# iris-ua/iris_lama

Measured on NVIDIA H100. Metric: scans/sec at 256 particles x 1080 beams, higher is better.
Workload: dtype f64

## Files before the change

iris_lama_b200/csrc/brushfire_warp.cuh:

```cuda
#pragma once

#include "ddm_core.h"
#include "device_store.cuh"

namespace lama_b200 {

constexpr unsigned kFullMask = 0xffffffffu;

struct SmemHeap {
    uint64_t* slot;
    uint32_t size, cap;

    __device__ __forceinline__ bool push(uint64_t value)
    {
        if (size >= cap) return false;
        int hole = (int)size++;
        while (hole > 0) {
            int parent = (hole - 1) >> 1;
            uint64_t pv = slot[parent + 1];
            if (!heap_comp(pv, value)) break;
            slot[hole + 1] = pv;
            hole = parent;
        }
        slot[hole + 1] = value;
        return true;
    }
    __device__ __forceinline__ uint64_t top() const { return slot[1]; }
    __device__ __forceinline__ uint64_t pop()
    {
        const uint64_t t = slot[1];
        const uint32_t last = --size;
        if (last == 0) return t;
        const uint64_t value = slot[last + 1];
        const int len = (int)last;
        int hole = 0, second = 0;
        const int lim = (len - 1) >> 1;
        while (second < lim) {
            second = 2 * (second + 1);
            const ulonglong2 ch = *reinterpret_cast<const ulonglong2*>(slot + second);
            uint64_t pick = ch.y;
            if (heap_comp(ch.y, ch.x)) {
                pick = ch.x;
                second--;
            }
            slot[hole + 1] = pick;
            hole = second;
        }
        if ((len & 1) == 0 && second == ((len - 2) >> 1)) {
            second = 2 * (second + 1);
            slot[hole + 1] = slot[second];
            hole = second - 1;
        }
        while (hole > 0) {
            int parent = (hole - 1) >> 1;
            uint64_t pv = slot[parent + 1];
            if (!heap_comp(pv, value)) break;
            slot[hole + 1] = pv;
            hole = parent;
        }
        slot[hole + 1] = value;
        return t;
    }
};

struct WarpBrushfire {
    const StoreView& s;
    int32_t* dir;
    int32_t* gdir;
    uint32_t* scratch;
    const uint32_t side;
    const int log2dim;
    const int lane;
    SmemHeap lower_q, raise_q;
    const uint32_t max_sqdist;
    uint32_t err;
    bool dead;
#ifdef LAMA_PHASE_TIMING
    long long cyc[6] = {0, 0, 0, 0, 0, 0};
#define BF_CLK(v) const long long v = clock64()
#define BF_ACC(k, a, b) cyc[k] += (b) - (a)
#else
#define BF_CLK(v) do { } while (0)
#define BF_ACC(k, a, b) do { } while (0)
#endif

    __device__ WarpBrushfire(const StoreView& sv, int32_t* d, int32_t* g, uint32_t* sc, int l, SmemHeap lo, SmemHeap ra, uint32_t msq)
        : s(sv), dir(d), gdir(g), scratch(sc), side((uint32_t)sv.window.dim * kPatchLen), log2dim(ilog2(sv.window.dim)), lane(l), lower_q(lo),
          raise_q(ra), max_sqdist(msq), err(0), dead(false) {}

    __host__ __device__ static int ilog2(int v)
    {
        int l = 0;
        while ((1 << (l + 1)) <= v) ++l;
        return l;
    }
    __device__ __forceinline__ static uint32_t key_of(uint32_t x, uint32_t y) { return (y << 16) | (x & 0xFFFFu); }
    __device__ __forceinline__ int dindex(uint32_t x, uint32_t y) const
    {
        return (x < side && y < side) ? (int)(((y >> kPatchLog2) << log2dim) | (x >> kPatchLog2)) : -1;
    }
    __device__ __forceinline__ uint32_t* cellptr(int entry, uint32_t x, uint32_t y) const
    {
        return s.pool + ((((uint32_t)entry & (uint32_t)kDirSlotMask) << (2 * kPatchLog2)) | cell_index(x, y));
    }

    __device__ __forceinline__ bool entry_ready(int e) const { return e >= 0 && (e & kDirOwn); }

    __device__ __forceinline__ bool ensure(int di)
    {
        int slot = warp_make_exclusive(s, dir, gdir, di, lane);
        if (slot < 0) {
            err |= kErrPoolEmpty;
            dead = true;
            return false;
        }
        return true;
    }
    __device__ __forceinline__ uint32_t* uptr(uint32_t x, uint32_t y)
    {
        const int di = dindex(x, y);
        if (di < 0 || dead) {
            if (di < 0) err |= kErrWindow;
            scratch[lane] = 0;
            return &scratch[lane];
        }
        int e = dir[di];
        if (!entry_ready(e)) {
            if (!ensure(di)) {
                scratch[lane] = 0;
                return &scratch[lane];
            }
            e = dir[di];
        }
        return cellptr(e, x, y);
    }
    __device__ __forceinline__ uint32_t* lptr(uint32_t x, uint32_t y, bool active)
    {
        const int di = active ? dindex(x, y) : -1;
        if (active && di < 0) err |= kErrWindow;
        int e = di >= 0 ? dir[di] : -1;
        unsigned m = __ballot_sync(kFullMask, di >= 0 && !entry_ready(e));
        while (m && !dead) {
            const int l = __ffs(m) - 1;
            ensure(__shfl_sync(kFullMask, di, l));
            e = di >= 0 ? dir[di] : -1;
            m = __ballot_sync(kFullMask, di >= 0 && !entry_ready(e));
        }
        if (!entry_ready(e) || dead) {
            scratch[lane] = 0;
            return &scratch[lane];
        }
        return cellptr(e, x, y);
    }
    __device__ __forceinline__ static bool same_patch(uint32_t x, uint32_t y, int dx, int dy)
    {
        return (uint32_t)((int)(x & (kPatchLen - 1)) + dx) < (uint32_t)kPatchLen && (uint32_t)((int)(y & (kPatchLen - 1)) + dy) < (uint32_t)kPatchLen;
    }
    __device__ __forceinline__ uint32_t* rel_uptr(uint32_t* base, uint32_t x, uint32_t y, int dx, int dy)
    {
        if (same_patch(x, y, dx, dy) && !is_scratch(base)) return base + dx + dy * kPatchLen;
        return uptr(x + dx, y + dy);
    }
    __device__ __forceinline__ uint32_t* rel_lptr(uint32_t* base, bool interior, uint32_t x, uint32_t y, int dx, int dy, bool active)
    {
        if (interior && !is_scratch(base)) return active ? base + dx + dy * kPatchLen : &scratch[lane];
        return lptr(x + dx, y + dy, active);
    }
    __device__ __forceinline__ bool is_scratch(const uint32_t* p) const { return p >= scratch && p < scratch + 32; }
    __device__ __forceinline__ static bool interior_cell(uint32_t x, uint32_t y)
    {
        return ((x & (kPatchLen - 1)) - 1u) < (uint32_t)(kPatchLen - 2) && ((y & (kPatchLen - 1)) - 1u) < (uint32_t)(kPatchLen - 2);
    }

    __device__ __forceinline__ uint32_t touch(uint32_t* p)
    {
        uint32_t w = *p;
        if (!(w & kDmKnown)) {
            w |= kDmKnown;
            *p = w;
        }
        return w;
    }

    __device__ __forceinline__ void push_lower(uint32_t prio, uint32_t key)
    {
        if (!lower_q.push(heap_entry(prio, key))) err |= kErrHeapOverflow;
    }
    __device__ __forceinline__ void push_raise(uint32_t prio, uint32_t key)
    {
        if (!raise_q.push(heap_entry(prio, key))) err |= kErrHeapOverflow;
    }

    __device__ __forceinline__ void add_obstacle(uint32_t x, uint32_t y)
    {
        uint32_t* c = uptr(x, y);
        const uint32_t w = touch(c);
        if ((w & kDmValid) && dm_sqdist(w) == 0) return;
        *c = dm_pack(0, 0, 0, true, true);
        push_lower(0, key_of(x, y));
    }
    __device__ __forceinline__ void remove_obstacle(uint32_t x, uint32_t y)
    {
        uint32_t* c = uptr(x, y);
        const uint32_t w = touch(c);
        if (!((w & kDmValid) && dm_sqdist(w) == 0)) return;
        *c = dm_pack(0, 0, 0, false, true);
        push_raise(0, key_of(x, y));
    }

    __device__ __forceinline__ void raise(uint32_t x, uint32_t y, uint32_t* cur)
    {
        const int i = lane & 3;
        const bool act = lane < 4;
        const int dxi = (i == 0) - (i == 2), dyi = (i == 1) - (i == 3);
        const uint32_t nx = x + dxi, ny = y + dyi;
        uint32_t* p = rel_lptr(cur, interior_cell(x, y), x, y, dxi, dyi, act);
        uint32_t n = 0;
        if (act) n = touch(p);
        const bool go = act && !((n & kDmQueued) || !(n & kDmValid));
        uint32_t* po = lptr(nx + dm_ox(n), ny + dm_oy(n), go);
        if (go) touch(po);
        __syncwarp();
        const uint32_t key = key_of(nx, ny);
        for (int j = 0; j < 4; ++j) {
            uint32_t o = 0;
            if (lane == j && go) o = *po;
            const bool g   = __shfl_sync(kFullMask, (int)go, j) != 0;
            if (!g) continue;
            const bool clr = __shfl_sync(kFullMask, (int)!(o & kDmValid), j) != 0;
            const uint32_t k  = __shfl_sync(kFullMask, key, j);
            const uint32_t pr = __shfl_sync(kFullMask, dm_sqdist(n), j);
            if (clr) {
                push_raise(pr, k);
                if (lane == j) *p = dm_pack(0, 0, 0, false, true);
            } else {
                push_lower(pr, k);
                if (lane == j) *p = n | kDmQueued;
            }
            __syncwarp();
        }
        if (lane == 0) *cur &= ~kDmQueued;
        __syncwarp();
    }

    __device__ __forceinline__ void lower(uint32_t x, uint32_t y, uint32_t* cur, uint32_t c)
    {
        const int cox = dm_ox(c), coy = dm_oy(c);
        const int i = lane & 3;
        const int dxi = (i == 0) - (i == 2), dyi = (i == 1) - (i == 3);
        const bool go = lane < 4 && !(dxi * cox > 0 || dyi * coy > 0);
        const uint32_t nx = x + dxi, ny = y + dyi;
        BF_CLK(c0);
        uint32_t* p = rel_lptr(cur, interior_cell(x, y), x, y, dxi, dyi, go);
        uint32_t n = 0;
        if (go) n = touch(p);
#ifdef LAMA_PHASE_TIMING
        n = __shfl_sync(kFullMask, n, lane);
#endif
        BF_CLK(c1);
        BF_ACC(2, c0, c1);
        const int rx = cox - dxi, ry = coy - dyi;
        const uint32_t new_sq = (uint32_t)(rx * rx + ry * ry);
        const uint32_t cmp_sq = (n & kDmValid) ? dm_sqdist(n) : max_sqdist;
        bool over = go && new_sq < cmp_sq;
        const bool chk = go && !over && new_sq == dm_sqdist(n);
        if (__any_sync(kFullMask, chk)) {
            uint32_t* po = lptr(nx + dm_ox(n), ny + dm_oy(n), chk);
            if (chk) {
                const uint32_t o = touch(po);
                if (!(n & kDmValid) || !((o & kDmValid) && dm_sqdist(o) == 0)) over = true;
            }
        }
        __syncwarp();
        unsigned m = __ballot_sync(kFullMask, over) & 0xFu;
        BF_CLK(c2);
        BF_ACC(3, c1, c2);
        const uint32_t key = key_of(nx, ny);
        while (m) {
            const int l = __ffs(m) - 1;
            m &= m - 1;
            BF_CLK(c4);
            push_lower(__shfl_sync(kFullMask, new_sq, l), __shfl_sync(kFullMask, key, l));
            BF_CLK(c5);
            BF_ACC(5, c4, c5);
            if (lane == l) *p = dm_pack(new_sq, rx, ry, true, true);
        }
        if (lane == 0) *cur = c & ~kDmQueued;
        __syncwarp();
        BF_CLK(c3);
        BF_ACC(4, c2, c3);
    }

    __device__ __forceinline__ uint32_t update()
    {
        uint32_t processed = 0;
        while (raise_q.size) {
            const uint32_t key = heap_key(raise_q.pop());
            const uint32_t x = key & 0xFFFFu, y = key >> 16;
            uint32_t* cur = uptr(x, y);
            touch(cur);
            ++processed;
            raise(x, y, cur);
        }
        while (lower_q.size) {
            BF_CLK(a0);
            const uint32_t key = heap_key(lower_q.pop());
            BF_CLK(a1);
            BF_ACC(0, a0, a1);
            const uint32_t x = key & 0xFFFFu, y = key >> 16;
            uint32_t* cur = uptr(x, y);
            const uint32_t c = touch(cur);
            ++processed;
            if (c & kDmValid) {
                const uint32_t o = touch(rel_uptr(cur, x, y, dm_ox(c), dm_oy(c)));
                BF_CLK(a2);
                BF_ACC(1, a1, a2);
                if (dm_sqdist(o) == 0 && (c & kDmQueued)) lower(x, y, cur, c);
            }
        }
        return processed;
    }
};

}
```

iris_lama_b200/csrc/kernels.cu:

```cuda
#include "kernels.cuh"

#include <cstdio>

#include "brushfire_warp.cuh"

namespace lama_b200 {

namespace {

constexpr int kMatchThreads = 576;
constexpr int kRayThreads   = 512;

__device__ __forceinline__ double warp_sum(double v)
{
#pragma unroll
    for (int o = 16; o > 0; o >>= 1) v += __shfl_xor_sync(0xffffffffu, v, o);
    return v;
}

struct MatchShared {
    uint64_t bar;
    Affine tf;
    SE2 state;
    SolverControl ctl;
// ... 1048 lines not shown
    const RayPullView& pv = rp.pull;
    const RayPullLayout L(rp.scan.n_beams);
    PullCtaShared& sh   = *reinterpret_cast<PullCtaShared*>(smem_raw);
    PullEntry* list     = reinterpret_cast<PullEntry*>(smem_raw + L.list);
    uint32_t* hits      = reinterpret_cast<uint32_t*>(smem_raw + L.hits);
    PullWarpShared& w   = reinterpret_cast<PullWarpShared*>(smem_raw + L.warps)[warp];
    const RayPullHeader* hdr = &sh.hdr;
    const int dim = s.window.dim, S = pv.splits;
    int log2dim = 0;
    while ((1 << (log2dim + 1)) <= dim) ++log2dim;
    if (tid == 0) mbar_init(&sh.bar, 1);
    uint32_t err = 0, parity = 0;
    for (;;) {
        __syncthreads();
        if (tid == 0) sh.unit = atomicAdd(pv.ctrl + 1, 1);
        __syncthreads();
        const int unit = sh.unit;
        if (unit >= count * S) break;
        const int pl = unit / S, split = unit - pl * S;
        if (!__ldcg(&pv.hdr[pl].ok)) continue;
        if (tid == 0) {
            sh.hdr  = pv.hdr[pl];
            sh.next = 0;
            const uint32_t b0 = (uint32_t)sh.hdr.prefix[8] * (uint32_t)sizeof(PullEntry), b1 = ((uint32_t)sh.hdr.n_hits * 4u + 15u) & ~15u;
            mbar_expect_tx(&sh.bar, b0 + b1);
            if (b0) tma_load_1d(list, pv.list + (size_t)pl * pv.stride, b0, &sh.bar);
            if (b1) tma_load_1d(hits, pv.hits + (size_t)pl * pv.stride, b1, &sh.bar);
        }
        mbar_wait(&sh.bar, parity);
        parity ^= 1u;
        __syncthreads();
        const int n_tasks = hdr->n_tasks, ox = hdr->ox, oy = hdr->oy;
        int32_t* gdir = dir_of(s, rp.set, rp.particle_offset + pl, kMapOcc);
        for (;;) {
            int t = 0;
            if (lane == 0) t = atomicAdd(&sh.next, 1);
            t = __shfl_sync(0xffffffffu, t, 0);
            const int ti = split + t * S;
            if (ti >= n_tasks) break;
            const uint2 task = __ldg(pv.tasks + hdr->task_base + ti);
            const int di = (int)(task.x & 0xFFFFu), h_lo = (int)(task.y >> 16), h_hi = h_lo + (int)(task.y & 0xFFFFu);
            const int px = di & (dim - 1), py = di >> log2dim;
            const int cx0 = px * kPatchLen - ox, cy0 = py * kPatchLen - oy;
            {
                uint32_t* tz = reinterpret_cast<uint32_t*>(w.tile);
#pragma unroll
                for (int i = 0; i < kPatchLen * kTileStride / 2 / 32; ++i) tz[i * 32 + lane] = 0u;
            }
            w.hitbits[lane] = 0u;
            __syncwarp();
            bool touched = false;
            {
                const int m = cx0 + lane;
                const uint32_t a = (uint32_t)(m < 0 ? -m : m);
                pull_patch_classes(list, hdr->prefix, 0, cx0, cy0, [&](int, bool mneg, bool tneg, int lo, int hi) {
                    if (m == 0 || (m < 0) != mneg) return;
                    for (int i = lo; i < hi; ++i) {
                        const int pos = pull_land(list[i], a, tneg, cy0);
                        if (pos >= 0) {
                            ++w.tile[pos * kTileStride + lane];
                            touched = true;
                        }
                    }
                });
            }
            __syncwarp();
            {
                const int m = cy0 + lane;
                const uint32_t a = (uint32_t)(m < 0 ? -m : m);
                pull_patch_classes(list, hdr->prefix, 4, cy0, cx0, [&](int, bool mneg, bool tneg, int lo, int hi) {
                    if (m == 0 || (m < 0) != mneg) return;
                    for (int i = lo; i < hi; ++i) {
                        const int pos = pull_land(list[i], a, tneg, cx0);
                        if (pos >= 0) {
                            ++w.tile[lane * kTileStride + pos];
                            touched = true;
                        }
                    }
                });
            }
            for (int i = h_lo + lane; i < h_hi; i += 32) {
                const uint32_t cell = pull_hit_cell(hits[i]);
                atomicOr(&w.hitbits[cell >> 5], 1u << (cell & 31));
            }
            __syncwarp();
            if (!__any_sync(0xffffffffu, touched) && h_hi == h_lo) continue;

            const int e0 = gdir[di];
            const bool hot = e0 >= 0 && (e0 & kDirHot);
            const int slot = warp_make_exclusive(s, gdir, gdir, di, lane);
            if (slot < 0) {
                err |= kErrPoolEmpty;
                continue;
            }
            uint32_t* patch = patch_ptr(s, slot);
            const uint32_t hitrow  = w.hitbits[lane];
            const uint32_t candrow = hitrow | (hot ? __ldcg(fbits_ptr(s, slot) + lane) : 0u);
            int ncand = 0;
            bool newhot = false;
            auto replay_candidates = [&]() {
                newhot |= pull_replay_patch<kProb>(s, rp, list, hdr->prefix, hits, h_lo, h_hi, w.cand, ncand, patch, slot, cx0, cy0, px, py, stats + pl,
                                                   events_out + (size_t)pl * rp.event_cap, lane);
                ncand = 0;
            };
            for (int r0 = 0; r0 < kPatchLen; r0 += 8) {
                uint32_t v[8];
#pragma unroll
                for (int k = 0; k < 8; ++k) v[k] = __ldcg(patch + (r0 + k) * kPatchLen + lane);
#pragma unroll
                for (int k = 0; k < 8; ++k) {
                    const int r = r0 + k;
                    const uint32_t cnt = w.tile[r * kTileStride + lane];
                    const uint32_t cw = __shfl_sync(0xffffffffu, candrow, r);
                    bool plain = cnt != 0u;
                    if (cw != 0u) {
                        const uint32_t hw = __shfl_sync(0xffffffffu, hitrow, r);
                        const bool iscand = (cw >> lane) & 1u, touch = cnt != 0u || ((hw >> lane) & 1u);
                        plain = touch && !iscand;
                        const uint32_t m = __ballot_sync(0xffffffffu, touch && iscand);
                        if (m) {
                            if (ncand + 32 > kPullCandCap) replay_candidates();
                            if (touch && iscand) w.cand[ncand + __popc(m & ((1u << lane) - 1u))] = (uint16_t)(r * kPatchLen + lane);
                            ncand += __popc(m);
                        }
                    }
                    if (plain) {
                        uint32_t* cell = patch + r * kPatchLen + lane;
                        if (!kProb) {
                            *cell = v[k] + (cnt << 16);
                        } else {
                            float p = __uint_as_float(v[k]);
                            for (uint32_t q = cnt; q > 0; --q) p = prob_miss(p, rp.prob);
                            *cell = __float_as_uint(p);
                        }
                    }
                    if (kProb) {
                        const uint32_t known = __ballot_sync(0xffffffffu, plain);
                        if (lane == 0 && known) kbits_ptr(s, slot)[r] |= known;
                    }
                }
            }
            __syncwarp();
            if (ncand) replay_candidates();
            if (__any_sync(0xffffffffu, newhot) && !hot && lane == 0) gdir[di] |= kDirHot;
            __syncwarp();
        }
    }
    err = __reduce_or_sync(0xffffffffu, err);
    if (lane == 0 && err) atomicOr(s.status, err);
}

constexpr int kBrushThreads = 128;
__global__ void __launch_bounds__(kBrushThreads)
k_brushfire(StoreView s, BrushParams bp, const uint64_t* __restrict__ events, MapUpdateStats* __restrict__ stats)
{
    extern __shared__ __align__(16) unsigned char smem_raw[];
    const int dim2    = s.window.dim * s.window.dim;
    int32_t* dir      = reinterpret_cast<int32_t*>(smem_raw);
    uint64_t* lower_h = reinterpret_cast<uint64_t*>(smem_raw + (size_t)dim2 * 4);
    uint64_t* raise_h = lower_h + bp.lower_cap + 2;
    uint64_t* ev      = raise_h + bp.raise_cap + 2;
    uint32_t* scratch = reinterpret_cast<uint32_t*>(ev + bp.event_cap);
    uint64_t* bar     = reinterpret_cast<uint64_t*>(scratch + 32);
    const int tid = threadIdx.x, lane = tid & 31, warp = tid >> 5, nwarps = blockDim.x >> 5;
    const int particle = bp.particle_offset + blockIdx.x;
    int32_t* gdir      = dir_of(s, bp.set, particle, kMapDm);

#ifdef LAMA_PHASE_TIMING
    long long bt[5] = {clock64(), 0, 0, 0, 0};
#endif
    if (tid == 0) mbar_init(bar, 1);
    __syncthreads();
    uint32_t nev = stats[blockIdx.x].events;
    uint32_t my_err = 0;
    if (nev > (uint32_t)bp.event_cap) {
        my_err |= kErrPushOverflow;
        nev = (uint32_t)bp.event_cap;
    }
    const uint64_t* gev = events + (size_t)blockIdx.x * bp.event_cap;
    const int evpad = next_pow2((int)nev);
    for (int i = tid; i < evpad; i += blockDim.x) ev[i] = i < (int)nev ? gev[i] : ~0ull;
    __syncthreads();
    block_bitonic_sort(ev, evpad);
    block_stage_tma(dir, gdir, (uint32_t)dim2 * 4u, bar, 0);

    {
        int reach = 0;
        while ((uint32_t)(reach * reach) < bp.max_sqdist) ++reach;
        const int dim = s.window.dim;
        for (uint32_t i = warp; i < nev; i += nwarps) {
            const uint32_t key = (uint32_t)ev[i];
            const int x = (int)(key & 0xFFFFu), y = (int)(key >> 16);
            const int px = x >> kPatchLog2, py = y >> kPatchLog2, cx = x & (kPatchLen - 1), cy = y & (kPatchLen - 1);
            const int x0 = cx < reach ? -1 : 0, x1 = cx >= kPatchLen - reach ? 1 : 0, y0 = cy < reach ? -1 : 0, y1 = cy >= kPatchLen - reach ? 1 : 0;
            for (int dy = y0; dy <= y1; ++dy)
                for (int dx = x0; dx <= x1; ++dx) {
                    const int qx = px + dx, qy = py + dy;
                    if ((unsigned)qx >= (unsigned)dim || (unsigned)qy >= (unsigned)dim) continue;
                    const int e = dir[qy * dim + qx];
                    if (e < 0) continue;
                    const uint32_t* row = patch_ptr(s, e & kDirSlotMask) + lane * kPatchLen;
                    asm volatile("prefetch.global.L1 [%0];" ::"l"(row));
                }
        }
    }
    if (warp != 0) return;
#ifdef LAMA_PHASE_TIMING
    bt[1] = clock64();
#endif

    WarpBrushfire bf(s, dir, gdir, scratch, lane, SmemHeap{lower_h, 0u, (uint32_t)bp.lower_cap}, SmemHeap{raise_h, 0u, (uint32_t)bp.raise_cap},
                     bp.max_sqdist);
    bf.err |= my_err;
    for (uint32_t i = 0; i < nev; ++i) {
        const uint64_t e   = ev[i];
        const uint32_t key = (uint32_t)e;
        if ((e >> 32) & 1u) bf.add_obstacle(key & 0xFFFFu, key >> 16);
        else bf.remove_obstacle(key & 0xFFFFu, key >> 16);
    }
#ifdef LAMA_PHASE_TIMING
    bt[2] = clock64();
    const uint32_t q0 = bf.raise_q.size, q1 = bf.lower_q.size;
#endif
    const uint32_t processed = bf.update();
#ifdef LAMA_PHASE_TIMING
    bt[3] = clock64();
    if (lane == 0 && bp.debug) printf("bf %d: pre %lld events %lld update %lld | nev %u raise %u lower %u pops %u\n", blockIdx.x, bt[1] - bt[0], bt[2] - bt[1], bt[3] - bt[2], nev, q0, q1, processed);
    if (lane == 0 && bp.debug) printf("bfc %d: pop %lld cur %lld nbr %lld chk %lld commit %lld (pushes %lld)\n", blockIdx.x, bf.cyc[0], bf.cyc[1], bf.cyc[2], bf.cyc[3], bf.cyc[4], bf.cyc[5]);
#endif
    const uint32_t err = __reduce_or_sync(0xffffffffu, bf.err);
    if (lane == 0) {
        stats[blockIdx.x].dm_pops = processed;
        if (err) atomicOr(s.status, err);
    }
}

__global__ void k_copy_dirs(StoreView s, int src_set, int dst_set, const int32_t* __restrict__ idx, int dst_first)
{
    const int p = dst_first + blockIdx.x, kind = blockIdx.y;
    const int dim2 = s.window.dim * s.window.dim;
    const int a  = idx[blockIdx.x];
    int32_t* src = dir_of(s, src_set, a < 0 ? 0 : a, kind);
    int32_t* dst = dir_of(s, dst_set, p, kind);
    for (int e = threadIdx.x; e < dim2; e += blockDim.x) {
        int slot = a < 0 ? -1 : src[e];
        if (slot >= 0) {
            atomicAdd(&s.refcount[slot & kDirSlotMask], 1);
            if ((slot & kDirOwn) && src_set == dst_set) src[e] = slot & ~kDirOwn;
            slot &= ~kDirOwn;
        }
        dst[e] = slot;
    }
}
__global__ void k_release(StoreView s, int set, int first)
{
    const int p = first + blockIdx.x, kind = blockIdx.y;
    const int dim2 = s.window.dim * s.window.dim;
    int32_t* d = dir_of(s, set, p, kind);
    for (int e = threadIdx.x; e < dim2; e += blockDim.x) {
        int slot = d[e];
        if (slot >= 0) {
            release_slot(s, slot & kDirSlotMask);
            d[e] = -1;
        }
    }
}
__global__ void k_delete_patches(StoreView s, int set, int particle, const int32_t* __restrict__ list)
{
    const int di = list[blockIdx.x];
    if (threadIdx.x != 0) return;
    for (int kind = 0; kind < s.n_kinds; ++kind) {
        int32_t* d = dir_of(s, set, particle, kind);
        const int e = d[di];
        if (e >= 0) {
            release_slot(s, e & kDirSlotMask);
            d[di] = -1;
        }
    }
}

__global__ void k_pack_results(const MatchResult* __restrict__ res, int n, double digest, double* __restrict__ out)
{
    const int i = blockIdx.x * blockDim.x + threadIdx.x;
    if (i < n) {
        const MatchResult& r = res[i];
        double* o = out + (size_t)i * kShardFields;
        o[0] = r.state.c; o[1] = r.state.s; o[2] = r.state.tx; o[3] = r.state.ty;
        o[4] = r.sums[11];
        o[5] = (double)r.evals_ref;
        o[6] = (double)r.iterations;
    }
    if (i == 0) out[(size_t)n * kShardFields] = digest;
}

__global__ void k_merge_free(StoreView s)
{
    __shared__ int n, base;
    if (threadIdx.x == 0) {
        n    = *s.freed_count;
        base = *s.free_count;
    }
    __syncthreads();
    for (int i = threadIdx.x; i < n; i += blockDim.x) s.free_slots[base + i] = s.freed[i];
    __syncthreads();
    if (threadIdx.x == 0) {
        *s.free_count  = base + n;
        *s.freed_count = 0;
        s.ray_ctrl[0] = s.ray_ctrl[1] = 0;
    }
}
__global__ void k_init_store(StoreView s, int n_sets)
{
    const size_t total_dir = (size_t)n_sets * s.n_particles * s.n_kinds * s.window.dim * s.window.dim;
    for (size_t i = blockIdx.x * (size_t)blockDim.x + threadIdx.x; i < total_dir; i += (size_t)gridDim.x * blockDim.x) s.dirs[i] = -1;
    for (size_t i = blockIdx.x * (size_t)blockDim.x + threadIdx.x; i < (size_t)s.n_slots; i += (size_t)gridDim.x * blockDim.x) {
        s.free_slots[i] = s.n_slots - 1 - (int)i;
        s.refcount[i]   = 0;
    }
    if (blockIdx.x == 0 && threadIdx.x == 0) {
        *s.free_count  = s.n_slots;
        *s.freed_count = 0;
        *s.status      = 0;
        s.counters[0] = s.counters[1] = s.counters[2] = 0;
    }
}

__global__ void k_export(StoreView s, int set, int particle, int kind, uint32_t x0, uint32_t y0, int w, int h, uint32_t* __restrict__ out,
                         uint8_t* __restrict__ present)
{
    const int32_t* d = dir_of(s, set, particle, kind);
    for (int k = blockIdx.x * blockDim.x + threadIdx.x; k < w * h; k += gridDim.x * blockDim.x) {
        uint32_t x = x0 + (uint32_t)(k % w), y = y0 + (uint32_t)(k / w);
        int di   = dir_index(s.window, x, y);
        int slot = di < 0 ? -1 : d[di];
        out[k]   = slot < 0 ? 0u : __ldcg(patch_ptr(s, slot & kDirSlotMask) + cell_index(x, y));
        if (present) present[k] = slot >= 0;
    }
}

__global__ void k_gather_cells(StoreView s, int set, int particle, int kind, const uint32_t* __restrict__ cells, int n, uint32_t* __restrict__ words,
                               uint8_t* __restrict__ flags)
{
    const int32_t* d = dir_of(s, set, particle, kind);
    for (int k = blockIdx.x * blockDim.x + threadIdx.x; k < n; k += gridDim.x * blockDim.x) {
        const uint32_t x = cells[2 * k], y = cells[2 * k + 1];
        const int di   = dir_index(s.window, x, y);
        const int slot = di < 0 ? -1 : d[di];
        uint32_t w = 0;
        uint8_t f = 0;
        if (slot >= 0) {
            const uint32_t ci = cell_index(x, y);
            w = __ldcg(patch_ptr(s, slot & kDirSlotMask) + ci);
            f = 1;
            if (kind == kMapOcc && s.kbits && ((__ldcg(kbits_ptr(s, slot & kDirSlotMask) + (ci >> 5)) >> (ci & 31)) & 1u)) f |= 2;
        }
        words[k] = w;
        flags[k] = f;
    }
}

__global__ void k_export_bits(StoreView s, int plane, int set, int particle, uint32_t x0, uint32_t y0, int w, int h, uint8_t* __restrict__ out)
{
    const int32_t* d = dir_of(s, set, particle, kMapOcc);
    for (int k = blockIdx.x * blockDim.x + threadIdx.x; k < w * h; k += gridDim.x * blockDim.x) {
        uint32_t x = x0 + (uint32_t)(k % w), y = y0 + (uint32_t)(k / w);
        int di   = dir_index(s.window, x, y);
        int slot = di < 0 ? -1 : d[di];
        uint8_t v = 0;
        const uint32_t* base = plane == 0 ? s.fbits : s.kbits;
        if (slot >= 0 && base) {
            const uint32_t ci = cell_index(x, y);
            v = (__ldcg(base + (size_t)(slot & kDirSlotMask) * 32 + (ci >> 5)) >> (ci & 31)) & 1u;
        }
        out[k] = v;
    }
}

__global__ void k_import(StoreView s, int set, int particle, int kind, uint32_t x0, uint32_t y0, int w, int h, const uint32_t* __restrict__ in)
{
    const int lane = threadIdx.x & 31;
    const int pw = w / kPatchLen, ph = h / kPatchLen;
// ... 192 lines not shown
        touch(tx | (ty << 16), kOccHitInc);
        if (!p.full) continue;
        if (bc.from[2] == bc.to[2]) {
            SegWalk w;
            w.init(fx, fy, tx, ty, 0, 1 << 30);
            while (w.next()) touch(w.P, kOccMissInc);
        } else {
            RayWalk3 w(bc);
            while (w.next()) touch((w.x - bx0) | ((w.y - by0) << 16), kOccMissInc);
        }
    }
    err = __reduce_or_sync(0xffffffffu, err);
    if ((threadIdx.x & 31) == 0 && err) atomicOr(s.status, err);
    if (!kMark) {
        for (int o = 16; o > 0; o >>= 1) cells += __shfl_xor_sync(0xffffffffu, cells, o);
        if ((threadIdx.x & 31) == 0 && cells) atomicAdd(p.cells, cells);
    }
}

__global__ void k_render_alloc(StoreView s, int set, const uint8_t* __restrict__ marks)
{
    const int lane = threadIdx.x & 31;
    const int di   = blockIdx.x * (blockDim.x >> 5) + (threadIdx.x >> 5);
    if (di >= s.window.dim * s.window.dim || !marks[di]) return;
    int32_t* dir = dir_of(s, set, 0, kMapOcc);
    if (dir[di] >= 0) return;
    int ns = 0;
    if (lane == 0) {
        ns = alloc_slot(s);
        if (ns >= 0) atomicAdd((unsigned long long*)&s.counters[0], 1ull);
    }
    ns = __shfl_sync(0xffffffffu, ns, 0);
    if (ns < 0) return;
    warp_zero_patch(patch_ptr(s, ns), lane);
    fbits_ptr(s, ns)[lane] = 0u;
    kbits_ptr(s, ns)[lane] = 0u;
    if (lane == 0) dir[di] = ns | kDirOwn;
}

__global__ void k_render_known(StoreView s, int set, uint8_t* __restrict__ marks)
{
    const int lane = threadIdx.x & 31;
    const int di   = blockIdx.x * (blockDim.x >> 5) + (threadIdx.x >> 5);
    if (di >= s.window.dim * s.window.dim || !marks[di]) return;
    const int e = dir_of(s, set, 0, kMapOcc)[di];
    if (e >= 0) {
        const uint32_t* cells = patch_ptr(s, e & kDirSlotMask);
        uint32_t* kb = kbits_ptr(s, e & kDirSlotMask);
        for (int row = 0; row < kPatchLen; ++row) {
            const uint32_t known = __ballot_sync(0xffffffffu, __ldcg(cells + row * kPatchLen + lane) != 0u);
            if (lane == 0 && known) kb[row] |= known;
        }
    }
    if (lane == 0) marks[di] = 0;
}

__global__ void k_prune_freq(StoreView s, int set)
{
    const int lane = threadIdx.x & 31;
    const int di   = blockIdx.x * (blockDim.x >> 5) + (threadIdx.x >> 5);
    if (di >= s.window.dim * s.window.dim) return;
    const int e = dir_of(s, set, 0, kMapOcc)[di];
    if (e < 0) return;
    uint32_t* cells = patch_ptr(s, e & kDirSlotMask);
    for (int row = 0; row < kPatchLen; ++row) {
        const uint32_t w = cells[row * kPatchLen + lane];
        if (occ_visited(w) == 1u && occ_occupied(w) <= 1u) cells[row * kPatchLen + lane] = 0u;
    }
}

}

size_t match_smem_bytes(int dir_dim, uint32_t max_sqdist)
{
    return (size_t)dir_dim * dir_dim * 4 + (size_t)(max_sqdist + 1) * 8 + ((sizeof(MatchShared) + 15) & ~(size_t)15) + (size_t)kNumSums * kMatchThreads * 8 + 16;
}
size_t raycast_smem_bytes(int dir_dim, const RayParams& rp)
{
    const int dim2 = dir_dim * dir_dim;
    const int n_groups = (rp.scan.n_beams + 31) / 32;
    const size_t beam_bytes = (size_t)n_groups * 32 * 16, ev_bytes = (size_t)rp.event_cap * 8;
    const size_t prob_extra = rp.prob_mode ? (size_t)dim2 * 4 + (size_t)((dim2 + 31) / 32) * 4 + 32 : 0;
    return (size_t)dim2 * 4 + (size_t)rp.log_cap * 8 + (beam_bytes > ev_bytes ? beam_bytes : ev_bytes) + (size_t)rp.cand_cap * 128 +
           (size_t)((dim2 + 31) / 32) * 8 + (size_t)(n_groups + 4) * 4 + (size_t)(rp.cand_cap + 4) * 2 + (size_t)dim2 * 4 + sizeof(RayShared) + 32 + prob_extra;
}
size_t brushfire_smem_bytes(int dir_dim, const BrushParams& bp)
{
    const int dim2 = dir_dim * dir_dim;
    return (size_t)dim2 * 4 + (size_t)(bp.lower_cap + bp.raise_cap + 4 + bp.event_cap) * 8 + 32 * 4 + 16 + 16;
}

template <typename Kernel>
static cudaError_t raise_smem_limit(Kernel* k, size_t bytes)
{
    cudaFuncAttributes a;
    cudaError_t e = cudaFuncGetAttributes(&a, k);
    if (e != cudaSuccess) return e;
    if ((size_t)a.maxDynamicSharedSizeBytes >= bytes) return cudaSuccess;
    return cudaFuncSetAttribute(k, cudaFuncAttributeMaxDynamicSharedMemorySize, (int)bytes);
}

cudaError_t configure_kernels(int dir_dim, uint32_t max_sqdist_limit, const RayParams& rp, const BrushParams& bp)
{
    cudaError_t e;
    e = raise_smem_limit(k_match, match_smem_bytes(dir_dim, max_sqdist_limit));
    if (e != cudaSuccess) return e;
    if (rp.prob_mode) e = raise_smem_limit(k_raycast<true>, raycast_smem_bytes(dir_dim, rp));
    else e = raise_smem_limit(k_raycast<false>, raycast_smem_bytes(dir_dim, rp));
    if (e != cudaSuccess) return e;
    e = raise_smem_limit(k_brushfire, brushfire_smem_bytes(dir_dim, bp));
    if (e != cudaSuccess) return e;
    e = raise_smem_limit(k_ray_setup, ray_setup_smem_bytes(dir_dim, rp.scan.n_beams > 4096 ? 4096 : rp.scan.n_beams));
    if (e != cudaSuccess) return e;
    e = raise_smem_limit(k_ray_pull<false>, ray_pull_smem_bytes(rp.scan.n_beams > 4096 ? 4096 : rp.scan.n_beams));
    if (e != cudaSuccess) return e;
    e = raise_smem_limit(k_ray_pull<true>, ray_pull_smem_bytes(rp.scan.n_beams > 4096 ? 4096 : rp.scan.n_beams));
    return e;
}

void launch_match(const StoreView& s, const MatchParams& mp, const SE2* d_states, MatchResult* d_results, int count, cudaStream_t st)
{
    if (count <= 0) return;
    const int n = mp.scan.n_beams, rounds = (n + kMatchThreads - 1) / kMatchThreads;
    int threads = (((n + rounds - 1) / rounds) + 31) & ~31;
    threads = threads < 128 ? 128 : threads;
    k_match<<<count, threads, match_smem_bytes(s.window.dim, mp.max_sqdist), st>>>(s, mp, d_states, d_results);
}
void launch_raycast(const StoreView& s, const RayParams& rp, const SE2* d_states, uint64_t* d_events, MapUpdateStats* d_stats, int count,
                    cudaStream_t st)
{
    if (count <= 0) return;
    if (rp.prob_mode) k_raycast<true><<<count, kRayThreads, raycast_smem_bytes(s.window.dim, rp), st>>>(s, rp, d_states, d_events, d_stats);
    else k_raycast<false><<<count, kRayThreads, raycast_smem_bytes(s.window.dim, rp), st>>>(s, rp, d_states, d_events, d_stats);
}
size_t ray_setup_smem_bytes(int dir_dim, int n_beams) { return RaySetupLayout(n_beams, dir_dim * dir_dim).total; }
size_t ray_pull_smem_bytes(int n_beams) { return RayPullLayout(n_beams).total; }
void launch_raycast_pull(const StoreView& s, const RayParams& rp_in, const SE2* d_states, uint64_t* d_events, MapUpdateStats* d_stats, int count, int n_sms,
                         cudaStream_t st)
{
    if (count <= 0) return;
    RayParams rp = rp_in;
    int splits = (6 * n_sms + count - 1) / count;
    rp.pull.splits = splits < 1 ? 1 : (splits > 64 ? 64 : splits);
    k_ray_setup<<<count, kSetupThreads, ray_setup_smem_bytes(s.window.dim, rp.scan.n_beams), st>>>(s, rp, d_states, d_stats);
    const int units = count * rp.pull.splits;
    const int grid = units < n_sms * kPullCtasPerSm ? units : n_sms * kPullCtasPerSm;
    const size_t smem = ray_pull_smem_bytes(rp.scan.n_beams);
    if (rp.prob_mode) k_ray_pull<true><<<grid, kPullWarps * 32, smem, st>>>(s, rp, count, d_events, d_stats);
    else k_ray_pull<false><<<grid, kPullWarps * 32, smem, st>>>(s, rp, count, d_events, d_stats);
}
void launch_brushfire(const StoreView& s, const BrushParams& bp, uint64_t* d_events, MapUpdateStats* d_stats, int count, cudaStream_t st)
{
    if (count <= 0) return;
    k_brushfire<<<count, kBrushThreads, brushfire_smem_bytes(s.window.dim, bp), st>>>(s, bp, d_events, d_stats);
}
void launch_copy_dirs(const StoreView& s, int src_set, int dst_set, const int32_t* d_idx, int dst_first, int count, cudaStream_t st)
{
    if (count <= 0) return;
    k_copy_dirs<<<dim3(count, 2), 256, 0, st>>>(s, src_set, dst_set, d_idx, dst_first);
}
void launch_release(const StoreView& s, int set, int first, int count, cudaStream_t st)
{
    if (count <= 0) return;
    k_release<<<dim3(count, s.n_kinds), 256, 0, st>>>(s, set, first);
}
void launch_merge_free(const StoreView& s, cudaStream_t st) { k_merge_free<<<1, 256, 0, st>>>(s); }
void launch_pack_results(const MatchResult* d_results, int n, double digest, double* d_out, cudaStream_t st)
{
    k_pack_results<<<(n + 127) / 128, 128, 0, st>>>(d_results, n, digest, d_out);
}
void launch_delete_patches(const StoreView& s, int set, int particle, const int32_t* d_list, int count, cudaStream_t st)
{
    if (count <= 0) return;
    k_delete_patches<<<count, 32, 0, st>>>(s, set, particle, d_list);
}
void launch_init_store(const StoreView& s, int n_sets, cudaStream_t st) { k_init_store<<<296, 256, 0, st>>>(s, n_sets); }
void launch_export(const StoreView& s, int set, int particle, int kind, uint32_t x0, uint32_t y0, int w, int h, uint32_t* d_out, uint8_t* d_present,
                   cudaStream_t st)
{
    int blocks = (w * h + 255) / 256;
    if (blocks > 1184) blocks = 1184;
    if (blocks < 1) blocks = 1;
    k_export<<<blocks, 256, 0, st>>>(s, set, particle, kind, x0, y0, w, h, d_out, d_present);
}
void launch_gather_cells(const StoreView& s, int set, int particle, int kind, const uint32_t* d_cells, int n, uint32_t* d_words, uint8_t* d_flags,
                         cudaStream_t st)
{
    if (n <= 0) return;
    k_gather_cells<<<(n + 255) / 256 < 592 ? (n + 255) / 256 : 592, 256, 0, st>>>(s, set, particle, kind, d_cells, n, d_words, d_flags);
}
void launch_export_bits(const StoreView& s, int plane, int set, int particle, uint32_t x0, uint32_t y0, int w, int h, uint8_t* d_out, cudaStream_t st)
{
    int blocks = (w * h + 255) / 256;
    if (blocks > 1184) blocks = 1184;
    if (blocks < 1) blocks = 1;
    k_export_bits<<<blocks, 256, 0, st>>>(s, plane, set, particle, x0, y0, w, h, d_out);
}
void launch_import(const StoreView& s, int set, int particle, int kind, uint32_t x0, uint32_t y0, int w, int h, const uint32_t* d_in, cudaStream_t st)
{
    int patches = (w / kPatchLen) * (h / kPatchLen);
    if (patches <= 0) return;
    k_import<<<(patches + 3) / 4, 128, 0, st>>>(s, set, particle, kind, x0, y0, w, h, d_in);
}
void launch_gather_patches(const StoreView& s, const int32_t* d_slots, int n, uint32_t* d_out, uint32_t* d_out_fbits, cudaStream_t st)
{
    if (n <= 0) return;
    k_gather_patches<<<(n + 3) / 4, 128, 0, st>>>(s, d_slots, n, d_out, d_out_fbits);
}
void launch_scatter_patches(const StoreView& s, int set, int particle, int kind, const int32_t* d_entries, int n, const uint32_t* d_in,
                            const uint32_t* d_in_fbits, cudaStream_t st)
{
    if (n <= 0) return;
    k_scatter_patches<<<(n + 3) / 4, 128, 0, st>>>(s, set, particle, kind, d_entries, n, d_in, d_in_fbits);
}
void launch_sampling(const StoreView& s, int set, int particle, const double* d_points, const ScanParams& scan, const SE2& pose, const double* d_offsets,
                     int n_offsets, int stride, double resolution, uint32_t max_sqdist, double* d_out, cudaStream_t st)
{
    if (n_offsets <= 0) return;
    k_sampling<<<n_offsets, 128, 0, st>>>(s, set, particle, d_points, scan, pose, d_offsets, stride, resolution, max_sqdist, d_out);
}
void launch_match_error(const StoreView& s, int set, int particle0, bool shared_map, const double* d_points, const ScanParams& scan, const SE2* d_states, int count,
                        double resolution, uint32_t max_sqdist, double* d_out, cudaStream_t st)
{
    if (count <= 0) return;
    k_match_error<<<count, 256, 0, st>>>(s, set, particle0, shared_map ? 1 : 0, d_points, scan, d_states, resolution, max_sqdist, d_out);
}
void launch_distance(const StoreView& s, int set, int particle, const double* d_pts, int n, double resolution, uint32_t max_sqdist, double* d_dist,
                     double* d_grad, cudaStream_t st)
{
    if (n <= 0) return;
    int blocks = (n + 255) / 256;
    if (blocks > 1184) blocks = 1184;
    k_distance<<<blocks, 256, 0, st>>>(s, set, particle, d_pts, n, resolution, max_sqdist, d_dist, d_grad);
}
void launch_render_scans(const StoreView& s, int set, const RenderParams& p, int n_scans, cudaStream_t st)
{
    if (n_scans <= 0) return;
    const int dim2 = s.window.dim * s.window.dim, blocks = (dim2 + 7) / 8;
    k_render_scans<true><<<n_scans, kRenderThreads, 0, st>>>(s, set, p);
    k_render_alloc<<<blocks, 256, 0, st>>>(s, set, p.marks);
    k_render_scans<false><<<n_scans, kRenderThreads, 0, st>>>(s, set, p);
    k_render_known<<<blocks, 256, 0, st>>>(s, set, p.marks);
}
void launch_prune_freq(const StoreView& s, int set, cudaStream_t st)
{
    const int dim2 = s.window.dim * s.window.dim;
    k_prune_freq<<<(dim2 + 7) / 8, 256, 0, st>>>(s, set);
}

}
```

Before: 1283.

## Batch brushfire lower-queue loads into fast owned-patch path and hint global pool

Restructures the lower-queue loop in the warp brushfire. When the patches involved are already owned, the current cell, its four neighbours and the obstacle cell are loaded together before the heap pop finishes, so memory latency overlaps with the heap sift. Otherwise it falls back to the old touch/lower path. It also passes the pool pointer as a separate kernel argument and asserts it is global memory, so the compiler can emit plain global loads instead of generic ones. The cost is more code paths and duplicated commit logic, and the known-bit marking must behave exactly like touch().

```diff
diff --git a/iris_lama_b200/csrc/brushfire_warp.cuh b/iris_lama_b200/csrc/brushfire_warp.cuh
--- a/iris_lama_b200/csrc/brushfire_warp.cuh
+++ b/iris_lama_b200/csrc/brushfire_warp.cuh
@@ -65,6 +65,7 @@
 
 struct WarpBrushfire {
     const StoreView& s;
+    uint32_t* const pool;
     int32_t* dir;
     int32_t* gdir;
     uint32_t* scratch;
@@ -76,7 +77,7 @@
     uint32_t err;
     bool dead;
 #ifdef LAMA_PHASE_TIMING
-    long long cyc[6] = {0, 0, 0, 0, 0, 0};
+    long long cyc[4] = {0, 0, 0, 0};
 #define BF_CLK(v) const long long v = clock64()
 #define BF_ACC(k, a, b) cyc[k] += (b) - (a)
 #else
@@ -84,9 +85,9 @@
 #define BF_ACC(k, a, b) do { } while (0)
 #endif
 
-    __device__ WarpBrushfire(const StoreView& sv, int32_t* d, int32_t* g, uint32_t* sc, int l, SmemHeap lo, SmemHeap ra, uint32_t msq)
-        : s(sv), dir(d), gdir(g), scratch(sc), side((uint32_t)sv.window.dim * kPatchLen), log2dim(ilog2(sv.window.dim)), lane(l), lower_q(lo),
-          raise_q(ra), max_sqdist(msq), err(0), dead(false) {}
+    __device__ WarpBrushfire(const StoreView& sv, uint32_t* pl, int32_t* d, int32_t* g, uint32_t* sc, int l, SmemHeap lo, SmemHeap ra, uint32_t msq)
+        : s(sv), pool(pl), dir(d), gdir(g), scratch(sc), side((uint32_t)sv.window.dim * kPatchLen), log2dim(ilog2(sv.window.dim)), lane(l),
+          lower_q(lo), raise_q(ra), max_sqdist(msq), err(0), dead(false) {}
 
     __host__ __device__ static int ilog2(int v)
     {
@@ -101,7 +102,9 @@
     }
     __device__ __forceinline__ uint32_t* cellptr(int entry, uint32_t x, uint32_t y) const
     {
-        return s.pool + ((((uint32_t)entry & (uint32_t)kDirSlotMask) << (2 * kPatchLog2)) | cell_index(x, y));
+        uint32_t* const p = pool + ((((uint32_t)entry & (uint32_t)kDirSlotMask) << (2 * kPatchLog2)) | cell_index(x, y));
+        __builtin_assume(__isGlobal(p));
+        return p;
     }
 
     __device__ __forceinline__ bool entry_ready(int e) const { return e >= 0 && (e & kDirOwn); }
@@ -250,15 +253,9 @@
         const int dxi = (i == 0) - (i == 2), dyi = (i == 1) - (i == 3);
         const bool go = lane < 4 && !(dxi * cox > 0 || dyi * coy > 0);
         const uint32_t nx = x + dxi, ny = y + dyi;
-        BF_CLK(c0);
         uint32_t* p = rel_lptr(cur, interior_cell(x, y), x, y, dxi, dyi, go);
         uint32_t n = 0;
         if (go) n = touch(p);
-#ifdef LAMA_PHASE_TIMING
-        n = __shfl_sync(kFullMask, n, lane);
-#endif
-        BF_CLK(c1);
-        BF_ACC(2, c0, c1);
         const int rx = cox - dxi, ry = coy - dyi;
         const uint32_t new_sq = (uint32_t)(rx * rx + ry * ry);
         const uint32_t cmp_sq = (n & kDmValid) ? dm_sqdist(n) : max_sqdist;
@@ -272,23 +269,25 @@
             }
         }
         __syncwarp();
+        commit(x, y, cur, c, p, over, new_sq, dm_pack(new_sq, rx, ry, true, true));
+    }
+
+    __device__ __forceinline__ void commit(uint32_t x, uint32_t y, uint32_t* cur, uint32_t c, uint32_t* p, bool over, uint32_t new_sq, uint32_t word)
+    {
+        const int i = lane & 3;
+        const uint32_t key = key_of(x + (i == 0) - (i == 2), y + (i == 1) - (i == 3));
         unsigned m = __ballot_sync(kFullMask, over) & 0xFu;
-        BF_CLK(c2);
-        BF_ACC(3, c1, c2);
-        const uint32_t key = key_of(nx, ny);
         while (m) {
             const int l = __ffs(m) - 1;
             m &= m - 1;
             BF_CLK(c4);
             push_lower(__shfl_sync(kFullMask, new_sq, l), __shfl_sync(kFullMask, key, l));
             BF_CLK(c5);
-            BF_ACC(5, c4, c5);
-            if (lane == l) *p = dm_pack(new_sq, rx, ry, true, true);
+            BF_ACC(3, c4, c5);
+            if (lane == l) *p = word;
         }
         if (lane == 0) *cur = c & ~kDmQueued;
         __syncwarp();
-        BF_CLK(c3);
-        BF_ACC(4, c2, c3);
     }
 
     __device__ __forceinline__ uint32_t update()
@@ -304,22 +303,78 @@
         }
         while (lower_q.size) {
             BF_CLK(a0);
-            const uint32_t key = heap_key(lower_q.pop());
-            BF_CLK(a1);
-            BF_ACC(0, a0, a1);
+            const uint32_t key = heap_key(lower_q.top());
             const uint32_t x = key & 0xFFFFu, y = key >> 16;
-            uint32_t* cur = uptr(x, y);
-            const uint32_t c = touch(cur);
+            const int i = lane & 3;
+            const int dxi = (i == 0) - (i == 2), dyi = (i == 1) - (i == 3);
+            const uint32_t nx = x + dxi, ny = y + dyi;
+            uint32_t* cur = dead ? nullptr : owned_ptr(x, y);
+            uint32_t* const np = (dead || lane >= 4) ? nullptr : owned_ptr(nx, ny);
+            uint32_t c = cur ? *cur : 0u;
+            const uint32_t nw = np ? *np : 0u;
+            lower_q.pop();
             ++processed;
-            if (c & kDmValid) {
-                const uint32_t o = touch(rel_uptr(cur, x, y, dm_ox(c), dm_oy(c)));
-                BF_CLK(a2);
-                BF_ACC(1, a1, a2);
-                if (dm_sqdist(o) == 0 && (c & kDmQueued)) lower(x, y, cur, c);
-            }
+            if (cur) {
+                if (!(c & kDmKnown)) {
+                    c |= kDmKnown;
+                    *cur = c;
+                }
+                BF_CLK(a1);
+                BF_ACC(0, a0, a1);
+                if (!(c & kDmValid)) continue;
+                const int cox = dm_ox(c), coy = dm_oy(c);
+                const bool go = lane < 4 && !(dxi * cox > 0 || dyi * coy > 0);
+                uint32_t* const op = same_patch(x, y, cox, coy) ? cur + cox + coy * kPatchLen : owned_ptr(x + cox, y + coy);
+                if (op && !__any_sync(kFullMask, go && !np)) {
+                    const uint32_t n = nw | kDmKnown;
+                    const int rx = cox - dxi, ry = coy - dyi;
+                    const uint32_t new_sq = (uint32_t)(rx * rx + ry * ry);
+                    const uint32_t cmp_sq = (n & kDmValid) ? dm_sqdist(n) : max_sqdist;
+                    bool over = go && new_sq < cmp_sq;
+                    const bool chk = go && !over && new_sq == dm_sqdist(n);
+                    const int nox = dm_ox(n), noy = dm_oy(n);
+                    uint32_t* qp = !chk ? nullptr : same_patch(nx, ny, nox, noy) ? np + nox + noy * kPatchLen : owned_ptr(nx + nox, ny + noy);
+                    const uint32_t o = *op;
+                    uint32_t q = qp ? *qp : 0u;
+                    if (!(o & kDmKnown)) *op = o | kDmKnown;
+                    BF_CLK(a2);
+                    BF_ACC(1, a1, a2);
+                    if (!(dm_sqdist(o) == 0 && (c & kDmQueued))) continue;
+                    if (__any_sync(kFullMask, chk && !qp)) {
+                        uint32_t* const p = lptr(nx + nox, ny + noy, chk && !qp);
+                        if (chk && !qp) {
+                            qp = p;
+                            q  = *p;
+                        }
+                    }
+                    if (go && !(nw & kDmKnown)) *np = n;
+                    if (chk) {
+                        if (!(q & kDmKnown)) *qp = q | kDmKnown;
+                        if (!(n & kDmValid) || !((q & kDmValid) && dm_sqdist(q) == 0)) over = true;
+                    }
+                    __syncwarp();
+                    commit(x, y, cur, c, np, over, new_sq, dm_pack(new_sq, rx, ry, true, true));
+                    BF_CLK(a3);
+                    BF_ACC(2, a2, a3);
+                    continue;
+                }
+            } else {
+                cur = uptr(x, y);
+                c   = touch(cur);
+                if (!(c & kDmValid)) continue;
+            }
+            const uint32_t o = touch(rel_uptr(cur, x, y, dm_ox(c), dm_oy(c)));
+            if (dm_sqdist(o) == 0 && (c & kDmQueued)) lower(x, y, cur, c);
         }
         return processed;
     }
+
+    __device__ __forceinline__ uint32_t* owned_ptr(uint32_t x, uint32_t y) const
+    {
+        const int di = dindex(x, y);
+        const int e  = di >= 0 ? dir[di] : -1;
+        return entry_ready(e) ? cellptr(e, x, y) : nullptr;
+    }
 };
 
 }
diff --git a/iris_lama_b200/csrc/kernels.cu b/iris_lama_b200/csrc/kernels.cu
--- a/iris_lama_b200/csrc/kernels.cu
+++ b/iris_lama_b200/csrc/kernels.cu
@@ -1224,7 +1224,7 @@
 
 constexpr int kBrushThreads = 128;
 __global__ void __launch_bounds__(kBrushThreads)
-k_brushfire(StoreView s, BrushParams bp, const uint64_t* __restrict__ events, MapUpdateStats* __restrict__ stats)
+k_brushfire(StoreView s, uint32_t* pool, BrushParams bp, const uint64_t* __restrict__ events, MapUpdateStats* __restrict__ stats)
 {
     extern __shared__ __align__(16) unsigned char smem_raw[];
     const int dim2    = s.window.dim * s.window.dim;
@@ -1281,8 +1281,8 @@
     bt[1] = clock64();
 #endif
 
-    WarpBrushfire bf(s, dir, gdir, scratch, lane, SmemHeap{lower_h, 0u, (uint32_t)bp.lower_cap}, SmemHeap{raise_h, 0u, (uint32_t)bp.raise_cap},
-                     bp.max_sqdist);
+    WarpBrushfire bf(s, pool, dir, gdir, scratch, lane, SmemHeap{lower_h, 0u, (uint32_t)bp.lower_cap},
+                     SmemHeap{raise_h, 0u, (uint32_t)bp.raise_cap}, bp.max_sqdist);
     bf.err |= my_err;
     for (uint32_t i = 0; i < nev; ++i) {
         const uint64_t e   = ev[i];
@@ -1298,7 +1298,7 @@
 #ifdef LAMA_PHASE_TIMING
     bt[3] = clock64();
     if (lane == 0 && bp.debug) printf("bf %d: pre %lld events %lld update %lld | nev %u raise %u lower %u pops %u\n", blockIdx.x, bt[1] - bt[0], bt[2] - bt[1], bt[3] - bt[2], nev, q0, q1, processed);
-    if (lane == 0 && bp.debug) printf("bfc %d: pop %lld cur %lld nbr %lld chk %lld commit %lld (pushes %lld)\n", blockIdx.x, bf.cyc[0], bf.cyc[1], bf.cyc[2], bf.cyc[3], bf.cyc[4], bf.cyc[5]);
+    if (lane == 0 && bp.debug) printf("bfc %d: trip1+sift %lld trip2 %lld commit %lld (pushes %lld)\n", blockIdx.x, bf.cyc[0], bf.cyc[1], bf.cyc[2], bf.cyc[3]);
 #endif
     const uint32_t err = __reduce_or_sync(0xffffffffu, bf.err);
     if (lane == 0) {
@@ -1797,7 +1797,7 @@
 void launch_brushfire(const StoreView& s, const BrushParams& bp, uint64_t* d_events, MapUpdateStats* d_stats, int count, cudaStream_t st)
 {
     if (count <= 0) return;
-    k_brushfire<<<count, kBrushThreads, brushfire_smem_bytes(s.window.dim, bp), st>>>(s, bp, d_events, d_stats);
+    k_brushfire<<<count, kBrushThreads, brushfire_smem_bytes(s.window.dim, bp), st>>>(s, s.pool, bp, d_events, d_stats);
 }
 void launch_copy_dirs(const StoreView& s, int src_set, int dst_set, const int32_t* d_idx, int dst_first, int count, cudaStream_t st)
 {
```

Result: faster. 1312, median of 6 (+2.3%).
